# lyndonchan/wsss-analysis

Measured on AMD Instinct MI355X. Metric: images/sec CAM+CRF pseudo-labels, VOC2012 321x321, higher is better.
Workload: dtype f16x3; 1 GPU; resnet50 CAM + dense-CRF (M=21, 10 mean-field iters), 321x321, batch 32 images (=64 samples) per GPU, image-sharded; batch_images=32, num_classes=20, parallelism=image-sharded x1, no collective, steps_per_rank=245

## Files before the change

include/wsscam.h:

```cpp
#ifndef WSSCAM_H
#define WSSCAM_H

#include <stddef.h>
#include <stdint.h>

#ifdef __cplusplus
extern "C" {
#endif

#define WSC_VERSION 100

typedef enum wsc_status {
    WSC_OK = 0,
    WSC_ERR_INVALID = -1,
    WSC_ERR_NO_DEVICE = -2,
    WSC_ERR_HIP = -3,
    WSC_ERR_MISSING_KEY = -4,
    WSC_ERR_SHAPE = -5,
    WSC_ERR_NOMEM = -6,
    WSC_ERR_KEY_RANGE = -7,
    WSC_ERR_CAPACITY = -8,
    WSC_ERR_RANGE = -9
} wsc_status;

typedef enum wsc_arch {
    WSC_ARCH_RESNET50_CAM = 0,
    WSC_ARCH_VGG16_CAM = 1,
    WSC_ARCH_M7_CAM = 2,
    WSC_ARCH_RESNET50_IRN = 3,
    WSC_ARCH_VGG16_IRN = 4,
    WSC_ARCH_M7_IRN = 5
} wsc_arch;

typedef enum wsc_precision {
    WSC_PREC_BF16 = 0,
    WSC_PREC_BF16X3 = 1,
    WSC_PREC_F16 = 2,
    WSC_PREC_F16X3 = 3
} wsc_precision;

typedef struct wsc_ctx wsc_ctx;
typedef struct wsc_net wsc_net;
typedef enum {
    WSC_OPT_CRF_GAUSS_ON_CHIP = 0,
    WSC_OPT_CRF_FUSED_BLUR = 1,
    WSC_OPT_CRF_BLUR_ON_CHIP = 2,
    WSC_OPT_CRF_RANK_BALLOT = 3,
    WSC_OPT_CRF_EMBED_FULL = 4,
    WSC_OPT_RW_TILED = 5,
    WSC_OPT_STEM_POOL_FUSED = 6,
    WSC_OPT_CONV_WINDOW = 7,
    WSC_OPT_CAM_HEAD_STREAM = 8,
    WSC_OPT_CRF_MSG_IN_UPDATE = 9,
    WSC_OPT_COUNT = 10
} wsc_option;

typedef struct wsc_crf wsc_crf;
typedef struct wsc_crf_v wsc_crf_v;

typedef struct wsc_tensor_desc {
    const char *name;
    const float *data;
    int32_t ndim;
    int64_t shape[4];
} wsc_tensor_desc;


int wsc_version(void);
const char *wsc_last_error(void);

int wsc_ctx_create(int device, void *stream, wsc_ctx **out);
void wsc_ctx_destroy(wsc_ctx *ctx);
int wsc_ctx_set_option(wsc_ctx *ctx, int option, int value);
int wsc_sync(wsc_ctx *ctx);
int wsc_ctx_range_status(wsc_ctx *ctx, int *flag_out, int clear);
int wsc_ctx_wait(wsc_ctx *ctx, wsc_ctx *other);
int wsc_ctx_mark(wsc_ctx *ctx, int slot);
int wsc_ctx_wait_mark(wsc_ctx *ctx, int slot);
int wsc_ctx_wait_for_mark(wsc_ctx *ctx, wsc_ctx *other, int slot);
int wsc_device_info(wsc_ctx *ctx, char *arch_name, size_t arch_name_len, int *num_cus);

int wsc_malloc(wsc_ctx *ctx, size_t bytes, void **dptr_out);
int wsc_free(wsc_ctx *ctx, void *dptr);
int wsc_memcpy_h2d(wsc_ctx *ctx, void *dst_dev, const void *src_host, size_t bytes);
int wsc_memcpy_d2h(wsc_ctx *ctx, void *dst_host, const void *src_dev, size_t bytes);
int wsc_memset(wsc_ctx *ctx, void *dst_dev, int value, size_t bytes);
int wsc_host_alloc(wsc_ctx *ctx, size_t bytes, void **host_out);
int wsc_host_free(wsc_ctx *ctx, void *host);
int wsc_host_write_segments(const char *path, int n, const void *const *ptrs, const size_t *sizes);
int wsc_memcpy_h2d_async(wsc_ctx *ctx, void *dst_dev, const void *src_pinned_host, size_t bytes);
int wsc_memcpy_d2h_async(wsc_ctx *ctx, void *dst_pinned_host, const void *src_dev, size_t bytes);

int wsc_timer_begin(wsc_ctx *ctx);
int wsc_timer_end(wsc_ctx *ctx, float *ms_out);

int wsc_profile_begin(wsc_ctx *ctx);
int wsc_profile_end(wsc_ctx *ctx, int max_classes, int32_t *calls_out, float *total_ms_out, double *work_out,
                    int *n_classes_out);
const char *wsc_profile_class_name(int cls);


int wsc_net_create(wsc_ctx *ctx, int arch, const wsc_tensor_desc *weights, int n_weights,
                   int num_classes, int precision, wsc_net **out);
void wsc_net_destroy(wsc_net *net);
int wsc_net_cam_size(const wsc_net *net, int S, int *h_out);
int wsc_net_feat_channels(const wsc_net *net, int *f_out);

int wsc_net_forward_cam(wsc_ctx *ctx, const wsc_net *net, const float *x_dev, int B, int S,
                        float *cam_dev, float *score_dev);
int wsc_net_cam_size_hw(const wsc_net *net, int H, int W, int *h_out, int *w_out);
int wsc_net_forward_cam_hw(wsc_ctx *ctx, const wsc_net *net, const float *x_dev, int B, int H, int W, float *cam_dev,
                           float *score_dev);

int wsc_net_forward_features(wsc_ctx *ctx, const wsc_net *net, const float *x_dev ,
                             int N, int S, float *feat_dev);

int wsc_net_forward_edge(wsc_ctx *ctx, const wsc_net *net, const float *x_dev, int B, int S, int feat_h, int feat_w,
                         float *edge_dev, float *dp_dev);

int wsc_rw_propagate(wsc_ctx *ctx, const float *x_dev, const float *edge_dev, int K, int h, int w,
                     const int32_t *dirs_host, const int32_t *path_start_host, const int32_t *path_yx_host, int D,
                     float beta, int n_steps, float *rw_dev);
int wsc_rw_propagate_batch(wsc_ctx *ctx, int n_img, const int32_t *K_host, const int32_t *h_host,
                           const int32_t *w_host, const float *x_dev, const float *edge_dev,
                           const int32_t *dirs_host, const int32_t *path_start_host, const int32_t *path_yx_host,
                           int D, float beta, int n_steps, float *rw_dev);

int wsc_net_forward_gradcam(wsc_ctx *ctx, const wsc_net *net, const float *x_dev, int N, int S, int relu,
                            float *cams_dev, float *score_dev);

#define WSC_CONV_GENERIC 0x100
int wsc_conv2d_nchw(wsc_ctx *ctx, const float *x_dev, int N, int Cin, int H, int W, const float *w_host,
                    int Cout, int kh, int kw, int stride, int pad, const float *scale_host,
                    const float *shift_host, const float *residual_dev, int relu, int precision,
                    float *y_dev);


// ... 90 lines not shown
```

wsss-analysis_amd/csrc/common.h:

```cpp
#pragma once
#include <hip/hip_runtime.h>
#include <stdint.h>
#include <map>
#include <string>
#include <unordered_map>
#include <vector>

#include "../../include/wsscam.h"

typedef uint16_t bf16_t;

typedef __bf16 bf16x8_t __attribute__((ext_vector_type(8)));
typedef _Float16 f16x8_t __attribute__((ext_vector_type(8)));
typedef float f32x16_t __attribute__((ext_vector_type(16)));
typedef float f32x4_t __attribute__((ext_vector_type(4)));

__host__ __device__ inline bf16_t f32_to_bf16(float f) {
    union { float f; uint32_t u; } v;
    v.f = f;
    uint32_t u = v.u;
    if ((u & 0x7fffffffu) > 0x7f800000u) return (bf16_t)((u >> 16) | 0x40);
    u += 0x7fffu + ((u >> 16) & 1u);
    return (bf16_t)(u >> 16);
}
// ... 28 lines not shown
    }
    return (uint16_t)(o | (sign >> 16));
#endif
}
__host__ __device__ inline float f16_to_f32(uint16_t h) {
#if defined(__HIP_DEVICE_COMPILE__)
    return (float)__builtin_bit_cast(_Float16, h);
#else
    union { float f; uint32_t u; } o, magic;
    magic.u = 113u << 23;
    const uint32_t shifted_exp = 0x7c00u << 13;
    o.u = ((uint32_t)h & 0x7fffu) << 13;
    const uint32_t exp = shifted_exp & o.u;
    o.u += (127u - 15u) << 23;
    if (exp == shifted_exp) o.u += (128u - 16u) << 23;
    else if (exp == 0) { o.u += 1u << 23; o.f -= magic.f; }
    o.u |= ((uint32_t)h & 0x8000u) << 16;
    return o.f;
#endif
}
__host__ __device__ inline uint16_t f32_to_h16(float f, int fmt) { return fmt ? f32_to_f16(f) : f32_to_bf16(f); }
__host__ __device__ inline float h16_to_f32(uint16_t h, int fmt) { return fmt ? f16_to_f32(h) : bf16_to_f32(h); }

void wsc_set_error(const char *fmt, ...);
#define WSC_HIP(expr)                                                                          \
    do {                                                                                       \
        hipError_t _e = (expr);                                                                \
        if (_e != hipSuccess) {                                                                \
            wsc_set_error("%s:%d: %s failed: %s", __FILE__, __LINE__, #expr,                   \
                          hipGetErrorString(_e));                                              \
            return WSC_ERR_HIP;                                                                \
        }                                                                                      \
    } while (0)
#define WSC_CHECK(cond, code, ...)                                                             \
    do {                                                                                       \
        if (!(cond)) {                                                                         \
            wsc_set_error(__VA_ARGS__);                                                        \
            return (code);                                                                     \
        }                                                                                      \
    } while (0)
#define WSC_TRY(expr)                                                                          \
    do {                                                                                       \
        int _s = (expr);                                                                       \
        if (_s != WSC_OK) return _s;                                                           \
    } while (0)

enum WscKernelClass {
    WSC_K_CONV256 = 0,
    WSC_K_CONV128,
    WSC_K_CONV64,
    WSC_K_CONV_SMALLCIN,
    WSC_K_POOL_MISC,
    WSC_K_CAM_TAIL,
    WSC_K_CRF_BUILD,
    WSC_K_GAUSS_MSG,
    WSC_K_BLUR,
    WSC_K_SLICE_UPDATE,
    WSC_K_CRF_MISC,
    WSC_K_COUNT
};
struct WscProfRecord {
    int cls;
    double work;
    hipEvent_t e0, e1;
};

struct wsc_ctx {
    int device = 0;
    hipStream_t stream = nullptr;
    bool own_stream = false;
    int num_cus = 0;
    std::string arch;
    void *ws = nullptr;
    size_t ws_bytes = 0;
    static constexpr int PIN_SLOTS = 8;
    struct PinSlot {
        void *p = nullptr;
        size_t bytes = 0;
        hipEvent_t ev = nullptr;
        bool busy = false;
    };
    PinSlot pin_ring[PIN_SLOTS];
    int pin_next = 0;
    int opt[WSC_OPT_COUNT] = {1, 1, 1, 0, 0, -1, 1, 1, 1, 1};
    void *pinned = nullptr;
    size_t pinned_bytes = 0;
    void *zero_page = nullptr;
    unsigned *range_host = nullptr, *range_dev = nullptr;
    hipEvent_t pinned_ev = nullptr;
    bool pinned_busy = false;
    hipEvent_t ev0 = nullptr, ev1 = nullptr;
    hipEvent_t join_ev = nullptr;
    hipEvent_t marks[8] = {};
    bool mark_set[8] = {};
    hipStream_t aux_stream = nullptr;
    hipEvent_t fork_ev = nullptr, aux_done_ev = nullptr;
    bool profiling = false;
    std::vector<WscProfRecord> prof;
    std::vector<hipEvent_t> prof_pool;
    std::multimap<size_t, void *> free_blocks;
    std::unordered_map<void *, size_t> live_blocks;
    std::vector<std::pair<void *, void (*)(void *)>> attachments;
};
int wsc_ctx_workspace(wsc_ctx *ctx, size_t bytes, void **out);
int wsc_ctx_range_check(wsc_ctx *ctx);
__device__ __forceinline__ unsigned half2_at_ceiling(unsigned hw) { return (hw & 0x7fff7fffu) + 0x04010401u; }
struct WscKernelTimer {
    wsc_ctx *ctx;
    int idx = -1;
    WscKernelTimer(wsc_ctx *c, int cls, double work);
    ~WscKernelTimer();
};
int wsc_ctx_cached_alloc(wsc_ctx *ctx, size_t bytes, void **out);
void wsc_ctx_cached_free(wsc_ctx *ctx, void *p);
struct WscCachedGuard {
    wsc_ctx *ctx;
    void *p;
    WscCachedGuard(wsc_ctx *c, void *q) : ctx(c), p(q) {}
    WscCachedGuard(const WscCachedGuard &) = delete;
    WscCachedGuard &operator=(const WscCachedGuard &) = delete;
    void free_now() {
        if (p) wsc_ctx_cached_free(ctx, p);
        p = nullptr;
    }
    ~WscCachedGuard() { free_now(); }
};
int wsc_ctx_upload_small(wsc_ctx *ctx, void *dst_dev, const void *src_host, size_t bytes);

struct ConvLaunch {
    const bf16_t *x, *x_lo;
    const bf16_t *w;
    const float *s1, *b1;
    const float *s2, *b2;
    const bf16_t *res, *res_lo;
    bf16_t *y, *y_lo;
    float *y_f32;
    int N, H, W, Cin, Ho, Wo, Cout, CoutPad;
    int kh, kw, stride, pad;
    int relu;
    int small_cin;
    int split;
    int fmt;
    int generic;
    int ldy;
    const bf16_t *x2, *x2_lo;
    int H2, W2, C2, stride2;
};
int conv_igemm_launch(wsc_ctx *ctx, const ConvLaunch &p);
int launch_cam_head(wsc_ctx *ctx, const bf16_t *x, const bf16_t *x_lo, int M, int K, const bf16_t *w, int Kw, int CoutPad,
                    const float *s1, const float *b1, int C, int relu, float *y);

int launch_nchw_to_nhwc4(wsc_ctx *ctx, const float *x, int N, int H, int W, bf16_t *y, bf16_t *y_lo, int fmt);
void stem_pool_input_dims(int H, int W, int *Hp, int *Wp);
int launch_stem_pool(wsc_ctx *ctx, const bf16_t *x, const bf16_t *x_lo, int N, int H, int W, const bf16_t *w, int Kw, const float *s1,
                     const float *b1, int relu, bf16_t *y, bf16_t *y_lo);
int launch_gather_strided(wsc_ctx *ctx, const bf16_t *x, const bf16_t *x_lo, int N, int H, int W, int C, int stride, int Ho, int Wo,
                          bf16_t *y, bf16_t *y_lo, int ldy);
int launch_nchw_to_nhwc4_pad(wsc_ctx *ctx, const float *x, int N, int H, int W, int Hp, int Wp, int pad, bf16_t *y, bf16_t *y_lo,
                             int fmt);
int launch_maxpool(wsc_ctx *ctx, const bf16_t *x, const bf16_t *x_lo, int N, int H, int W, int C, int k,
                   int stride, int pad, int Ho, int Wo, bf16_t *y, bf16_t *y_lo, int fmt);
int launch_flip_add(wsc_ctx *ctx, const float *head, int B, int h, int w, int C, int Cs, float *cam);
int launch_gap_linear_sigmoid(wsc_ctx *ctx, const bf16_t *feat, const bf16_t *feat_lo, int B, int hw, int F,
                              const float *Wc, const float *bias, int C, float *score, int fmt,
                              int sample_stride);
int launch_bf16_to_f32(wsc_ctx *ctx, const bf16_t *x, const bf16_t *x_lo, size_t n, float *y, int fmt);
int launch_nchw_to_nhwc(wsc_ctx *ctx, const float *x, int N, int C, int HW, bf16_t *y, bf16_t *y_lo, int fmt);
// ... 12 lines not shown
```

wsss-analysis_amd/csrc/crf.hip:

```cpp
#include "common.h"

#include <atomic>
#include <cmath>
#include <cstring>

namespace {

constexpr unsigned long long EMPTY_KEY = 0xFFFFFFFFFFFFFFFFull;
typedef float f32x2_t __attribute__((ext_vector_type(2)));

struct LatticeDev {
    int d = 0;
    int rep = 1;
    int rows = 0;
    int32_t *offset = nullptr;
    float *bary = nullptr;
    float *norm = nullptr;
    int2 *nbr = nullptr;
    int32_t *tslot_start = nullptr;
    int2 *slot_desc = nullptr;
    float *tent_w = nullptr;
    uint8_t *tent_p = nullptr;
    int32_t *row_slot_start = nullptr;
    int n_tiles = 0, n_slots = 0;
// ... 1646 lines not shown
    const float *sw = T.tent_w + ebase_pix * T.dp1;
    const uint8_t *sp = T.tent_p + ebase_pix * T.dp1;
#pragma unroll
    for (int i = 0; i < EN; ++i) {
        const int e = (int)threadIdx.x + i * (int)blockDim.x;
        r.w[i] = 0.f;
        r.px[i] = 0u;
        if (e < ne) {
            r.w[i] = sw[e];
            r.px[i] = sp[e];
        }
    }
    r.desc = make_int2(0, 0);
    if ((int)threadIdx.x < r.s_end - r.s_beg && threadIdx.x < GATHER_SB) r.desc = T.slot_desc[r.s_beg + threadIdx.x];
}
template <int EN>
__device__ __forceinline__ void splat_commit(const SplatTab &T, int np, const SplatRegs<EN> &r, uint2 *lent, int2 *ldesc, int LP) {
    const int ne = (WSC_SPLAT_ABL & 4) ? 0 : np * T.dp1;
#pragma unroll
    for (int i = 0; i < EN; ++i) {
        const int e = (int)threadIdx.x + i * (int)blockDim.x;
        if (e < ne) lent[e] = make_uint2(r.px[i] * (unsigned)LP, __float_as_uint(r.w[i]));
    }
    if (threadIdx.x < GATHER_SB) ldesc[threadIdx.x] = r.desc;
}
__device__ __forceinline__ void tile_gather(const SplatTab &T, int s_beg, int s_end, int rep_k,
                                            const f32x4_t *stage, uint2 *lent, int2 *ldesc, int LP, int l, int g, int gpw,
                                            bool act) {
    f32x4_t *part = reinterpret_cast<f32x4_t *>(T.part) + (T.shared ? (size_t)rep_k * T.n_slots * LP : (size_t)0);
    const int nw = (int)(blockDim.x >> 6), wv = (int)(threadIdx.x >> 6);
    for (int sb0 = s_beg; sb0 < s_end; sb0 += GATHER_SB) {
        const int nsb = min(GATHER_SB, s_end - sb0);
        if (sb0 > s_beg) {
            if ((int)threadIdx.x < nsb) ldesc[threadIdx.x] = T.slot_desc[sb0 + threadIdx.x];
            __syncthreads();
        }
        for (int s0 = wv * gpw; s0 < nsb; s0 += nw * gpw) {
            const int s = s0 + g;
            const bool ok = act && s < nsb;
            const int2 d = ok ? ldesc[s] : make_int2(0, 0);
            const int i0 = d.x & 0xffff, n = (WSC_SPLAT_ABL & 2) ? 0 : d.x >> 16;
            f32x2_t a01 = {0.f, 0.f}, a23 = {0.f, 0.f};
            const uint2 *le = lent + i0;
            int i = 0;
            for (; i + 4 <= n; i += 4) {
                uint2 en[4];
                f32x4_t in[4];
#pragma unroll
                for (int jj = 0; jj < 4; ++jj) en[jj] = le[i + jj];
#pragma unroll
                for (int jj = 0; jj < 4; ++jj) in[jj] = stage[en[jj].x + l];
#pragma unroll
                for (int jj = 0; jj < 4; ++jj) {
                    const float w = __uint_as_float(en[jj].y);
                    const f32x2_t w2 = {w, w}, lo = {in[jj][0], in[jj][1]}, hi = {in[jj][2], in[jj][3]};
                    a01 = __builtin_elementwise_fma(w2, lo, a01);
                    a23 = __builtin_elementwise_fma(w2, hi, a23);
                }
            }
            if (i < n) {
                uint2 en[3];
                f32x4_t in[3];
#pragma unroll
                for (int jj = 0; jj < 3; ++jj) en[jj] = le[min(i + jj, n - 1)];
#pragma unroll
                for (int jj = 0; jj < 3; ++jj) in[jj] = stage[en[jj].x + l];
#pragma unroll
                for (int jj = 0; jj < 3; ++jj) {
                    const float w = i + jj < n ? __uint_as_float(en[jj].y) : 0.f;
                    const f32x2_t w2 = {w, w}, lo = {in[jj][0], in[jj][1]}, hi = {in[jj][2], in[jj][3]};
                    a01 = __builtin_elementwise_fma(w2, lo, a01);
                    a23 = __builtin_elementwise_fma(w2, hi, a23);
                }
            }
            const f32x4_t acc = {a01[0], a01[1], a23[0], a23[1]};
            if (ok && !(WSC_SPLAT_ABL & 1)) part[(unsigned)d.y * (unsigned)LP + l] = acc;
        }
        __syncthreads();
    }
}

constexpr int REC_LDS_BYTES = 56;
static_assert(TILE_PIX * REC_LDS_BYTES <= (int)(sizeof(uint2) * GATHER_ENT + sizeof(int2) * GATHER_SB), "record stage");
template <bool SLICE, bool SPLAT, bool GF = false, bool DMA = false, int FG = 0>
__global__ __launch_bounds__(512) __attribute__((amdgpu_waves_per_eu(4))) void update_splat_kernel(UpdateArgs a) {
    static_assert(!DMA || (SLICE && GF) || (!SLICE && SPLAT), "the LDS-DMA staging belongs to the GF updates and the first update");
    static_assert(FG == 0 || (SLICE && GF && DMA), "the in-kernel Gaussian message belongs to the DMA-staged GF updates");
    extern __shared__ f32x4_t stage[];
    const int LP = a.LP;
    const int gpw = 64 / LP;
    const int lane = threadIdx.x & 63;
    const int g = lane / LP;
    const int l = lane - g * LP;
    const bool act = g < gpw;
    const int seg0 = g * LP;
    const int nb = gridDim.x, bid = blockIdx.x;
    const int xcd = bid & 7, qq = nb >> 3, rr = nb & 7;
    const int lb = (xcd < rr ? xcd * (qq + 1) : rr * (qq + 1) + (xcd - rr) * qq) + (bid >> 3);
    const int k = lb / a.tg.tpi, j = lb - k * a.tg.tpi;
    const TileBox tb = tile_box(a.tg, j);
    const int np = tb.cw * tb.ch;
    const int N = a.tg.H * a.tg.W;
    const int ppt = (int)(blockDim.x >> 6) * gpw;
    const unsigned cw_magic = tile_div_magic(tb.cw);
    const size_t pix0 = (size_t)k * (size_t)N + (size_t)tb.y0 * (size_t)a.tg.W + (size_t)tb.x0;
    const unsigned LP16 = (unsigned)LP * 16u, l16 = (unsigned)l * 16u;
    constexpr unsigned REC_BYTES = GF ? 52u : 80u;
    constexpr int REC_ID = GF ? 0 : 3, REC_BARY = GF ? 6 : 12, REC_NORM = GF ? 12 : 19;
    const char *rec_b = (GF ? reinterpret_cast<const char *>(a.pix_rec_b) : reinterpret_cast<const char *>(a.pix_rec)) + pix0 * REC_BYTES;
    const char *u_b = reinterpret_cast<const char *>(a.u) + pix0 * LP16;
    char *q_b = reinterpret_cast<char *>(a.q) + pix0 * LP16;
    const char *vg_b = reinterpret_cast<const char *>(a.val_g) + (a.g_rows ? (size_t)k * a.g_rows * LP16 : (size_t)0);
    const char *vb_b = reinterpret_cast<const char *>(a.val_b);
    auto pixel_of = [&](int t0) -> unsigned {
        const int t = t0 + g;
        const unsigned tc = (act && t < np) ? (unsigned)t : 0u;
        const unsigned ty = (tc * cw_magic) >> 16, tx = tc - __umul24(ty, (unsigned)tb.cw);
        return __umul24(ty, (unsigned)a.tg.W) + tx;
    };
    uint4 rq[5];
    f32x4_t unn;
    f32x2_t e01, e23;
    const float cag = a.compat_g * a.alpha_g, cab = a.compat_b * a.alpha_b;
    const char *lrec = reinterpret_cast<const char *>(stage + TILE_PIX * LP);
    auto tile_idx = [&](int t0) -> unsigned {
        const int t = t0 + g;
        return (act && t < np) ? (unsigned)t : 0u;
    };
    auto load_u = [&](int t0) -> f32x4_t {
        if (DMA) return stage[tile_idx(t0) * (unsigned)LP + (unsigned)l];
        return ld_off<f32x4_t>(u_b, __umul24(pixel_of(t0), LP16) + l16);
    };
    auto load_rec = [&](int t0, uint4(&r)[5]) {
        if (DMA) {
            const char *q = lrec + tile_idx(t0) * (unsigned)REC_LDS_BYTES;
            uint2 w[6];
#pragma unroll
            for (int i = 0; i < 6; ++i) w[i] = *reinterpret_cast<const uint2 *>(q + 8 * i);
            r[0] = make_uint4(w[0].x, w[0].y, w[1].x, w[1].y);
            r[1] = make_uint4(w[2].x, w[2].y, w[3].x, w[3].y);
            r[2] = make_uint4(w[4].x, w[4].y, w[5].x, w[5].y);
            r[3] = make_uint4(*reinterpret_cast<const uint32_t *>(q + 48), 0u, 0u, 0u);
            r[4] = make_uint4(0u, 0u, 0u, 0u);
            return;
        }
        const unsigned p = pixel_of(t0);
        if (GF) {
#pragma unroll
            for (int i = 0; i < 3; ++i) r[i] = ld_off<uint4>(rec_b, __umul24(p, REC_BYTES) + 16u * i);
            r[3] = make_uint4(ld_off<uint32_t>(rec_b, __umul24(p, REC_BYTES) + 48u), 0u, 0u, 0u);
            r[4] = make_uint4(0u, 0u, 0u, 0u);
        } else {
#pragma unroll
            for (int i = 0; i < 5; ++i) r[i] = ld_off<uint4>(rec_b, __umul24(p, REC_BYTES) + 16u * i);
        }
    };
    auto issue_rows = [&](const uint4(&r)[5], f32x4_t(&g3)[3], f32x4_t(&b6)[6], float(&w9)[9]) {
        uint32_t rc[20];
#pragma unroll
        for (int i = 0; i < 5; ++i) {
            rc[4 * i] = r[i].x; rc[4 * i + 1] = r[i].y; rc[4 * i + 2] = r[i].z; rc[4 * i + 3] = r[i].w;
        }
        if (!GF) {
#pragma unroll
            for (int i = 0; i < 3; ++i) g3[i] = ld_off<f32x4_t>(vg_b, __umul24(rc[i], LP16) + l16);
        }
#pragma unroll
        for (int i = 0; i < 6; ++i) b6[i] = ld_off<f32x4_t>(vb_b, __umul24(rc[REC_ID + i], LP16) + l16);
        const float wb = cab * __uint_as_float(rc[REC_NORM]);
        if (!GF) {
// ... 180 lines not shown
            for (int it = 0; it < NIT; ++it) {
                const int i = tid + it * GM_THREADS;
                if (i < nitems) gl[i] = o[it];
            }
            __syncthreads();
        }
#pragma unroll
        for (int it = 0; it < NPI; ++it) {
            const int i = tid + it * GM_THREADS;
            if (i < np * LP) {
                const unsigned t = ((unsigned)i * lp_magic) >> 16, ll = (unsigned)i - t * (unsigned)LP;
                const uint4 gp = gpx[it];
                const f32x4_t uu = stage[i];
                f32x2_t o01 = {-uu[0], -uu[1]}, o23 = {-uu[2], -uu[3]};
                const float wr[3] = {__uint_as_float(gp.y) * cag, __uint_as_float(gp.z) * cag, __uint_as_float(gp.w) * cag};
#pragma unroll
                for (int r = 0; r < 3; ++r) {
                    const f32x4_t row = gl[((gp.x >> (10 * r)) & 1023u) * (unsigned)LP + ll];
                    const f32x2_t w2 = {wr[r], wr[r]}, lo = {row[0], row[1]}, hi = {row[2], row[3]};
                    o01 = __builtin_elementwise_fma(w2, lo, o01);
                    o23 = __builtin_elementwise_fma(w2, hi, o23);
                }
                stage[i] = f32x4_t{o01[0], o01[1], o23[0], o23[1]};
            }
        }
        if (SPLAT) splat_fetch<EN_G>(a.sg, a.sg.shared ? j : lb, (a.sg.shared ? 0ll : (long long)k * N) + tb.ebase, np, rg);
        __syncthreads();
    }
    WSC_TL(a, 4);
    auto emit = [&](int t0) {
        const int t = t0 + g;
        const bool ok = act && t < np;
        const unsigned p = pixel_of(t0);
        float e[4] = {e01[0], e01[1], e23[0], e23[1]};
        float mx = -3.0e38f;
#pragma unroll
        for (int kk = 0; kk < 4; ++kk) {
            e[kk] = (ok && 4 * l + kk < a.M) ? e[kk] : -3.0e38f;
            mx = fmaxf(mx, e[kk]);
        }
        for (int o = 4; o > 0; o >>= 1) {
            const float other = __shfl_down(mx, o, 64);
            if (l + o < LP) mx = fmaxf(mx, other);
        }
        mx = __shfl(mx, seg0, 64);
        float ex[4], sum = 0.f;
        const float mxl = mx * 1.44269504088896341f;
#pragma unroll
        for (int kk = 0; kk < 4; ++kk) {
            ex[kk] = __builtin_amdgcn_exp2f(__builtin_fmaf(e[kk], 1.44269504088896341f, -mxl));
            sum += ex[kk];
        }
        for (int o = 4; o > 0; o >>= 1) {
            const float other = __shfl_down(sum, o, 64);
            if (l + o < LP) sum += other;
        }
        sum = __shfl(sum, seg0, 64);
        const float rs = __builtin_amdgcn_rcpf(sum);
        const f32x4_t o4 = {ex[0] * rs, ex[1] * rs, ex[2] * rs, ex[3] * rs};
        if (ok) {
            if (SPLAT) stage[t * LP + l] = o4;
            if (a.q) *reinterpret_cast<f32x4_t *>(q_b + (__umul24(p, LP16) + l16)) = o4;
        }
        if (!SPLAT && a.argmax != nullptr) {
            float bv = o4[0];
            int bi = 4 * l;
#pragma unroll
            for (int kk = 1; kk < 4; ++kk)
                if (4 * l + kk < a.M && o4[kk] > bv) {
                    bv = o4[kk];
                    bi = 4 * l + kk;
                }
            for (int o = 4; o > 0; o >>= 1) {
                const float ov = __shfl_down(bv, o, 64);
                const int oi = __shfl_down(bi, o, 64);
                if (l + o < LP && ov > bv) {
                    bv = ov;
                    bi = oi;
                }
            }
            if (ok && l == 0) a.argmax[pix0 + p] = bi;
        }
    };
    {
        {
            const f32x4_t u0 = load_u(t_first);
            f32x4_t g3[3], b6[6];
            float w9[9];
            if (SLICE) {
                load_rec(t_first, rq);
                issue_rows(rq, g3, b6, w9);
            }
            unn = u0;
            if (t_first + ppt < np) {
                if (SLICE) load_rec(t_first + ppt, rq);
                unn = load_u(t_first + ppt);
            }
            fold(u0, g3, b6, w9, e01, e23);
        }
        for (int t0 = t_first; t0 < np; t0 += ppt) {
            const bool has_next = t0 + ppt < np;
            f32x4_t vgn[3], vbn[6];
            float wrn[9];
            const f32x4_t un1 = unn;
            if (SLICE && has_next) issue_rows(rq, vgn, vbn, wrn);
            if (t0 + 2 * ppt < np) {
                if (SLICE) load_rec(t0 + 2 * ppt, rq);
                unn = load_u(t0 + 2 * ppt);
            }
            emit(t0);
            if (has_next) fold(un1, vgn, vbn, wrn, e01, e23);
        }
    }
    WSC_TL(a, 5);
    if (SPLAT) {
        uint2 *lent = reinterpret_cast<uint2 *>(stage + TILE_PIX * LP);
        int2 *ldesc = reinterpret_cast<int2 *>(lent + GATHER_ENT);
        if (DMA) __syncthreads();
        splat_commit<EN_G>(a.sg, np, rg, lent, ldesc, LP);
        SplatRegs<EN_B> rb;
        splat_fetch<EN_B>(a.sb, a.sb.shared ? j : lb, (a.sb.shared ? 0ll : (long long)k * N) + tb.ebase, np, rb);
        __syncthreads();
        tile_gather(a.sg, rg.s_beg, rg.s_end, k, stage, lent, ldesc, LP, l, g, gpw, act);
        WSC_TL(a, 6);
        splat_commit<EN_B>(a.sb, np, rb, lent, ldesc, LP);
        __syncthreads();
        tile_gather(a.sb, rb.s_beg, rb.s_end, k, stage, lent, ldesc, LP, l, g, gpw, act);
    }
    WSC_TL(a, 7);
}

#ifndef WSC_GF_ABL
#define WSC_GF_ABL 0
#endif
struct GaussMsgArgs {
    const int4 *gt_cnt;
    const int2 *gt_rows;
    const uint4 *gt_nbr;
    const uint4 *gt_pix;
    const float *part;
    const float *u;
    float *e;
    int gt_stride, n_slots, shared, LP, B;
    float cag;
    TileGeom tg;
};
template <int NIT, int NPI>
__global__ __launch_bounds__(GM_THREADS) __attribute__((amdgpu_waves_per_eu(4))) void gauss_msg_kernel(GaussMsgArgs a) {
    extern __shared__ f32x4_t gl[];
    const int LP = a.LP, stride = a.gt_stride, tid = (int)threadIdx.x;
    const f32x4_t zero = {0.f, 0.f, 0.f, 0.f};
    const int nb = gridDim.x, bid = blockIdx.x;
    const int xcd = bid & 7, qq = nb >> 3, rr = nb & 7;
    const int lb = (xcd < rr ? xcd * (qq + 1) : rr * (qq + 1) + (xcd - rr) * qq) + (bid >> 3);
    const int k = lb / a.tg.tpi, j = lb - k * a.tg.tpi;
    const TileBox tb = tile_box(a.tg, j);
    const int np = tb.cw * tb.ch;
    const int N = a.tg.H * a.tg.W;
    unsigned *lnb = reinterpret_cast<unsigned *>(gl + (size_t)stride * (size_t)LP);
    const f32x4_t *partg = reinterpret_cast<const f32x4_t *>(a.part) + (a.shared ? (size_t)k * a.n_slots * LP : (size_t)0);
    const int nitems = stride * LP;
    const unsigned lp_magic = (65536u + (unsigned)LP - 1u) / (unsigned)LP;
    const unsigned cw_magic = tile_div_magic(tb.cw);
    const int2 *trow = a.gt_rows + (size_t)j * stride;
    const uint4 *tn = a.gt_nbr + (size_t)j * stride;
    const unsigned gpix0 = (unsigned)tb.y0 * (unsigned)a.tg.W + (unsigned)tb.x0;
    const size_t pix0 = (size_t)k * (size_t)N + gpix0;
// ... 671 lines not shown
                WSC_HIP(hipStreamSynchronize(ctx->stream));
                WSC_TRY(crf_alloc(crf, sizeof(int2) * nt * GBI * GBJ, (void **)&L.tile_pstart));
                hipLaunchKernelGGL(gauss_tile_pstart_kernel, dim3(grid1d(nt * GBI * GBJ)), dim3(256), 0, ctx->stream,
                                   L.tile_rows, L.row_slot_start, nt * GBI * GBJ, L.tile_pstart);
            }
        }
    }
    float *va, *vb, *vp;
    WSC_TRY(tmp.alloc(sizeof(float) * L.rows, (void **)&va));
    WSC_TRY(tmp.alloc(sizeof(float) * L.rows, (void **)&vb));
    WSC_TRY(tmp.alloc(sizeof(float) * (size_t)(L.n_slots + 1), (void **)&vp));
    splat_ones(ctx, L, make_geom(crf->H, crf->W), va, vp);
    float *res = blur_all1(ctx, L, va, vb);
    uint32_t *rec_b = nullptr;
    if (D == 5 && !shared && crf->lat[0].gt_rows && !crf->pix_rec_b) {
        WSC_TRY(crf_alloc(crf, sizeof(uint32_t) * 13 * (size_t)npix, (void **)&crf->pix_rec_b));
        rec_b = crf->pix_rec_b;
    }
    if (!shared && D == 5) {
        hipLaunchKernelGGL(slice_norm_tile_kernel, dim3((unsigned)L.n_tiles), dim3(256), 0, ctx->stream, L.offset, L.bary, dp1,
                           L.alpha, res, make_geom(crf->H, crf->W), L.norm, rec_b, L.tent_w, L.tent_p);
    } else {
        hipLaunchKernelGGL(slice_norm_kernel, dim3(grid1d(npix)), dim3(256), 0, ctx->stream, L.offset, L.bary, dp1,
                           L.alpha, res, npix, L.norm, rec_b);
        hipLaunchKernelGGL(tile_scale_entries_kernel, dim3((unsigned)L.n_tiles), dim3(256), 0, ctx->stream, L.norm, dp1,
                           make_geom(crf->H, crf->W), L.tent_w, L.tent_p);
    }
    WSC_HIP(hipGetLastError());
    return WSC_OK;
}

struct GaussCache {
    int H, W;
    float sxy;
    LatticeDev L;
    std::vector<void *> blocks;
    int users = 0;
    unsigned long long last_use = 0;
    bool fuse_pending = true;
};
constexpr int GAUSS_CACHE_MAX = 64;
std::atomic<unsigned long long> g_gauss_use_clock{0};
void gauss_cache_delete(void *p) { delete static_cast<GaussCache *>(p); }

int update_threads() {
#ifdef WSC_AB_KNOBS
    const char *te = getenv("WSC_CRF_UPD_THREADS");
    const int nthr = te ? atoi(te) : 256;
    return nthr == 512 ? 512 : 256;
#else
    return 256;
#endif
}
size_t update_splat_lds(int LP) { return sizeof(f32x4_t) * TILE_PIX * LP + sizeof(uint2) * GATHER_ENT + sizeof(int2) * GATHER_SB; }
size_t gauss_msg_lds(int LP, int gt_stride) { return ((size_t)LP * sizeof(f32x4_t) + sizeof(uint4)) * (size_t)gt_stride; }
bool update_gf_ok(const wsc_ctx *ctx, const LatticeDev &G, int LP) {
    if (!ctx->opt[WSC_OPT_CRF_GAUSS_ON_CHIP]) return false;
    if (!G.gt_rows || G.rep < 1 || G.gt_stride <= 0) return false;
    if ((long long)G.gt_stride * LP > 6ll * GM_THREADS || (long long)G.gt_stride * LP >= 8192) return false;
    return gauss_msg_lds(LP, G.gt_stride) <= 64 * 1024;
}

int launch_gauss_msg(wsc_ctx *ctx, hipStream_t st, const GaussMsgArgs &g, double bytes) {
    WscKernelTimer timer(ctx, WSC_K_GAUSS_MSG, bytes);
    const dim3 grid((unsigned)(g.B * g.tg.tpi)), block(GM_THREADS);
    size_t lds = gauss_msg_lds(g.LP, g.gt_stride);
#ifdef WSC_AB_KNOBS
    const char *le = getenv("WSC_CRF_GM_LDS");
    if (le && (size_t)atoi(le) > lds && atoi(le) <= 64 * 1024) lds = (size_t)atoi(le);
#endif
    if ((long long)g.gt_stride * g.LP <= 4ll * GM_THREADS && g.LP <= 6)
        hipLaunchKernelGGL((gauss_msg_kernel<4, 3>), grid, block, lds, st, g);
    else
        hipLaunchKernelGGL((gauss_msg_kernel<6, 4>), grid, block, lds, st, g);
    WSC_HIP(hipGetLastError());
    return WSC_OK;
}

size_t update_fg_lds(int LP, int gt_stride) { return update_splat_lds(LP) + gauss_msg_lds(LP, gt_stride); }
bool update_fg_ok(const wsc_ctx *ctx, const LatticeDev &G, int LP) {
    if (!ctx->opt[WSC_OPT_CRF_MSG_IN_UPDATE] || !update_gf_ok(ctx, G, LP)) return false;
    return update_fg_lds(LP, G.gt_stride) <= 80 * 1024;
}
int launch_update(wsc_ctx *ctx, const UpdateArgs &a, bool slice, bool splat, bool gf, bool fg = false, double fg_bytes = 0.0) {
    const double npix = (double)a.B * a.tg.H * a.tg.W;
    const double by = npix * (2.0 * a.M * 4 + (slice ? (gf ? 6 * 8 + 1.0 * a.M * 4 : 9 * 8 + 2.0 * a.M * 4) : 0.0) +
                              (splat ? 9 * 8 + 2.0 * a.M * 4 : 0.0));
    WscKernelTimer timer(ctx, WSC_K_SLICE_UPDATE, by + (fg ? fg_bytes : 0.0));
    const dim3 grid((unsigned)(a.B * a.tg.tpi)), block(update_threads());
    size_t lds = splat ? update_splat_lds(a.LP) : 0;
    if (fg) {
        const size_t l = update_fg_lds(a.LP, a.gt_stride);
        const bool small = (long long)a.gt_stride * a.LP <= 4ll * GM_THREADS && a.LP <= 6;
        auto set_lds = [&](const void *fn) {
            static bool done[64][4] = {};
            const int dev = ctx->device >= 0 && ctx->device < 64 ? ctx->device : 0, vi = (small ? 0 : 2) + (splat ? 0 : 1);
            if (!done[dev][vi] && l > 48 * 1024) {
                (void)hipFuncSetAttribute(fn, hipFuncAttributeMaxDynamicSharedMemorySize, 96 * 1024);
                done[dev][vi] = true;
            }
        };
        if (small) {
            if (splat) {
                set_lds(reinterpret_cast<const void *>(update_splat_kernel<true, true, true, true, 4>));
                hipLaunchKernelGGL((update_splat_kernel<true, true, true, true, 4>), grid, dim3(GM_THREADS), l, ctx->stream, a);
            } else {
                set_lds(reinterpret_cast<const void *>(update_splat_kernel<true, false, true, true, 4>));
                hipLaunchKernelGGL((update_splat_kernel<true, false, true, true, 4>), grid, dim3(GM_THREADS), l, ctx->stream, a);
            }
        } else {
            if (splat) {
                set_lds(reinterpret_cast<const void *>(update_splat_kernel<true, true, true, true, 6>));
                hipLaunchKernelGGL((update_splat_kernel<true, true, true, true, 6>), grid, dim3(GM_THREADS), l, ctx->stream, a);
            } else {
                set_lds(reinterpret_cast<const void *>(update_splat_kernel<true, false, true, true, 6>));
                hipLaunchKernelGGL((update_splat_kernel<true, false, true, true, 6>), grid, dim3(GM_THREADS), l, ctx->stream, a);
            }
        }
        WSC_HIP(hipGetLastError());
        return WSC_OK;
    }
#ifdef WSC_AB_KNOBS
    const char *de = getenv("WSC_CRF_UPD_DMA");
#else
    const char *de = nullptr;
#endif
    const bool dma = slice && gf && !(de && atoi(de) == 0);
    if (dma) lds = update_splat_lds(a.LP);
    if (dma) {
        if (splat) hipLaunchKernelGGL((update_splat_kernel<true, true, true, true>), grid, block, lds, ctx->stream, a);
        else hipLaunchKernelGGL((update_splat_kernel<true, false, true, true>), grid, block, lds, ctx->stream, a);
    } else if (slice && gf) {
        if (splat) hipLaunchKernelGGL((update_splat_kernel<true, true, true>), grid, block, lds, ctx->stream, a);
        else hipLaunchKernelGGL((update_splat_kernel<true, false, true>), grid, block, lds, ctx->stream, a);
    } else if (slice && splat) hipLaunchKernelGGL((update_splat_kernel<true, true>), grid, block, lds, ctx->stream, a);
    else if (slice) hipLaunchKernelGGL((update_splat_kernel<true, false>), grid, block, lds, ctx->stream, a);
    else if (splat && !(de && atoi(de) == 0))
        hipLaunchKernelGGL((update_splat_kernel<false, true, false, true>), grid, block, lds, ctx->stream, a);
    else if (splat) hipLaunchKernelGGL((update_splat_kernel<false, true>), grid, block, lds, ctx->stream, a);
    else hipLaunchKernelGGL((update_splat_kernel<false, false>), grid, block, lds, ctx->stream, a);
    WSC_HIP(hipGetLastError());
    return WSC_OK;
}

int crf_full_records(wsc_crf *crf, hipStream_t st) {
    if (crf->pix_rec) return WSC_OK;
    wsc_ctx *bctx = crf->ctx;
    WSC_TRY(crf_alloc(crf, sizeof(uint4) * 5 * (size_t)crf->B * crf->N, (void **)&crf->pix_rec));
    if (st != bctx->stream) {
        WSC_HIP(hipEventRecord(bctx->join_ev, bctx->stream));
        WSC_HIP(hipStreamWaitEvent(st, bctx->join_ev, 0));
    }
    hipLaunchKernelGGL(pack_pixels_kernel, dim3((unsigned)grid1d((long long)crf->N * 5, 256, 2048), (unsigned)crf->B), dim3(256), 0, st,
                       crf->lat[0].offset, crf->lat[0].bary, crf->lat[0].norm, crf->lat[1].offset, crf->lat[1].bary,
                       crf->lat[1].norm, crf->N, crf->lat[0].rep > 1 ? 1 : 0, crf->pix_rec);
    WSC_HIP(hipGetLastError());
    return WSC_OK;
}

int crf_bilateral_records(wsc_crf *crf, hipStream_t st) {
    if (crf->pix_rec_b) return WSC_OK;
    wsc_ctx *bctx = crf->ctx;
    WSC_TRY(crf_alloc(crf, sizeof(uint32_t) * 13 * (size_t)crf->B * crf->N, (void **)&crf->pix_rec_b));
    if (st != bctx->stream) {
        WSC_HIP(hipEventRecord(bctx->join_ev, bctx->stream));
        WSC_HIP(hipStreamWaitEvent(st, bctx->join_ev, 0));
    }
    hipLaunchKernelGGL(pack_pixels_b_kernel, dim3((unsigned)grid1d((long long)crf->B * crf->N * 13, 256, 8192)), dim3(256), 0, st,
                       crf->lat[1].offset, crf->lat[1].bary, crf->lat[1].norm, (long long)crf->B * crf->N, crf->pix_rec_b);
    WSC_HIP(hipGetLastError());
    return WSC_OK;
}

}

extern "C" {

int wsc_crf_create(wsc_ctx *ctx, const uint8_t *rgb_dev, int B, int H, int W, float g_sxy, float bi_sxy,
                   float bi_srgb, wsc_crf **out) {
    WSC_CHECK(ctx && rgb_dev && out, WSC_ERR_INVALID, "wsc_crf_create: null argument");
    WSC_CHECK(B > 0 && H > 0 && W > 0, WSC_ERR_INVALID, "wsc_crf_create: B=%d H=%d W=%d", B, H, W);
    WSC_CHECK(g_sxy > 0.f && bi_sxy > 0.f && bi_srgb > 0.f, WSC_ERR_INVALID,
              "wsc_crf_create: kernel widths must be positive");
    WSC_HIP(hipSetDevice(ctx->device));
    wsc_crf *crf = new wsc_crf();
    crf->ctx = ctx; crf->B = B; crf->H = H; crf->W = W; crf->N = H * W;
    WscKernelTimer timer(ctx, WSC_K_CRF_BUILD, (double)B * H * W * (3.0 * 16 + 6.0 * 16));
    int st = WSC_OK;
    GaussCache *hit = nullptr, *lru = nullptr;
    int n_cached = 0;
    size_t lru_at = 0;
    for (size_t i = 0; i < ctx->attachments.size(); ++i) {
        auto &a = ctx->attachments[i];
        if (a.second == &gauss_cache_delete) {
            ++n_cached;
            GaussCache *g = static_cast<GaussCache *>(a.first);
            if (g->H == H && g->W == W && g->sxy == g_sxy) hit = g;
            if (g->users == 0 && (!lru || g->last_use < lru->last_use)) {
                lru = g;
                lru_at = i;
// ... 382 lines not shown
```

wsss-analysis_amd/wsscam/_lib.py:

```python
import ctypes
import os
import re
import threading

import numpy as np

_HERE = os.path.dirname(os.path.abspath(__file__))
LIB_PATH = os.path.join(_HERE, "libwsscam.so")
HEADER_PATH = os.path.normpath(os.path.join(_HERE, "..", "..", "include", "wsscam.h"))

WSC_OK = 0
WSC_ERR_INVALID = -1
WSC_ERR_NO_DEVICE = -2
WSC_ERR_HIP = -3
WSC_ERR_MISSING_KEY = -4
WSC_ERR_SHAPE = -5
WSC_ERR_NOMEM = -6
WSC_ERR_KEY_RANGE = -7
WSC_ERR_CAPACITY = -8
WSC_ERR_RANGE = -9

ARCH_RESNET50_CAM = 0
ARCH_VGG16_CAM = 1
ARCH_M7_CAM = 2
ARCH_RESNET50_IRN = 3
ARCH_VGG16_IRN = 4
ARCH_M7_IRN = 5

PREC_BF16 = 0
PREC_BF16X3 = 1
PREC_F16 = 2
PREC_F16X3 = 3
OPT_CRF_GAUSS_ON_CHIP, OPT_CRF_FUSED_BLUR, OPT_CRF_BLUR_ON_CHIP, OPT_CRF_RANK_BALLOT, OPT_CRF_EMBED_FULL, OPT_RW_TILED, \
    OPT_STEM_POOL_FUSED, OPT_CONV_WINDOW, OPT_CAM_HEAD_STREAM, OPT_CRF_MSG_IN_UPDATE = range(10)
OPT_DEFAULTS = {OPT_CRF_GAUSS_ON_CHIP: 1, OPT_CRF_FUSED_BLUR: 1, OPT_CRF_BLUR_ON_CHIP: 1, OPT_CRF_RANK_BALLOT: 0,
                OPT_CRF_EMBED_FULL: 0, OPT_RW_TILED: -1, OPT_STEM_POOL_FUSED: 1, OPT_CONV_WINDOW: 1, OPT_CAM_HEAD_STREAM: 1,
                OPT_CRF_MSG_IN_UPDATE: 1}
CONV_GENERIC = 0x100


class WscError(RuntimeError):
    def __init__(self, status, message):
        super().__init__("libwsscam error %d: %s" % (status, message))
        self.status = status


class TensorDesc(ctypes.Structure):
    _fields_ = [
        ("name", ctypes.c_char_p),
        ("data", ctypes.POINTER(ctypes.c_float)),
        ("ndim", ctypes.c_int32),
        ("shape", ctypes.c_int64 * 4),
    ]


_lib = None

_vp = ctypes.c_void_p
_i = ctypes.c_int
_f = ctypes.c_float
_sz = ctypes.c_size_t

_SIGNATURES = {
    "wsc_version": (_i, []),
    "wsc_last_error": (ctypes.c_char_p, []),
    "wsc_ctx_create": (_i, [_i, _vp, ctypes.POINTER(_vp)]),
    "wsc_ctx_destroy": (None, [_vp]),
    "wsc_sync": (_i, [_vp]),
    "wsc_ctx_range_status": (_i, [_vp, ctypes.POINTER(_i), _i]),
    "wsc_ctx_wait": (_i, [_vp, _vp]),
    "wsc_ctx_mark": (_i, [_vp, _i]),
    "wsc_ctx_wait_mark": (_i, [_vp, _i]),
    "wsc_ctx_wait_for_mark": (_i, [_vp, _vp, _i]),
    "wsc_device_info": (_i, [_vp, ctypes.c_char_p, _sz, ctypes.POINTER(_i)]),
    "wsc_malloc": (_i, [_vp, _sz, ctypes.POINTER(_vp)]),
    "wsc_free": (_i, [_vp, _vp]),
    "wsc_memcpy_h2d": (_i, [_vp, _vp, _vp, _sz]),
    "wsc_memcpy_d2h": (_i, [_vp, _vp, _vp, _sz]),
    "wsc_memset": (_i, [_vp, _vp, _i, _sz]),
    "wsc_ctx_set_option": (_i, [_vp, _i, _i]),
    "wsc_host_alloc": (_i, [_vp, _sz, ctypes.POINTER(_vp)]),
    "wsc_host_free": (_i, [_vp, _vp]),
    "wsc_host_write_segments": (_i, [ctypes.c_char_p, _i, ctypes.POINTER(_vp), ctypes.POINTER(_sz)]),
    "wsc_memcpy_h2d_async": (_i, [_vp, _vp, _vp, _sz]),
    "wsc_memcpy_d2h_async": (_i, [_vp, _vp, _vp, _sz]),
    "wsc_profile_begin": (_i, [_vp]),
    "wsc_profile_end": (_i, [_vp, _i, _vp, _vp, _vp, ctypes.POINTER(_i)]),
    "wsc_profile_class_name": (ctypes.c_char_p, [_i]),
    "wsc_timer_begin": (_i, [_vp]),
    "wsc_timer_end": (_i, [_vp, ctypes.POINTER(_f)]),
    "wsc_net_create": (_i, [_vp, _i, ctypes.POINTER(TensorDesc), _i, _i, _i, ctypes.POINTER(_vp)]),
    "wsc_net_destroy": (None, [_vp]),
    "wsc_net_cam_size": (_i, [_vp, _i, ctypes.POINTER(_i)]),
    "wsc_net_feat_channels": (_i, [_vp, ctypes.POINTER(_i)]),
    "wsc_net_forward_cam": (_i, [_vp, _vp, _vp, _i, _i, _vp, _vp]),
    "wsc_net_forward_gradcam": (_i, [_vp, _vp, _vp, _i, _i, _i, _vp, _vp]),
    "wsc_net_forward_features": (_i, [_vp, _vp, _vp, _i, _i, _vp]),
    "wsc_net_cam_size_hw": (_i, [_vp, _i, _i, ctypes.POINTER(_i), ctypes.POINTER(_i)]),
    "wsc_net_forward_cam_hw": (_i, [_vp, _vp, _vp, _i, _i, _i, _vp, _vp]),
    "wsc_net_forward_edge": (_i, [_vp, _vp, _vp, _i, _i, _i, _i, _vp, _vp]),
    "wsc_rw_propagate": (_i, [_vp, _vp, _vp, _i, _i, _i, _vp, _vp, _vp, _i, _f, _i, _vp]),
    "wsc_rw_propagate_batch": (_i, [_vp, _i, _vp, _vp, _vp, _vp, _vp, _vp, _vp, _vp, _i, _f, _i, _vp]),
    "wsc_conv2d_nchw": (_i, [_vp, _vp, _i, _i, _i, _i, _vp, _i, _i, _i, _i, _i, _vp, _vp, _vp, _i, _i, _vp]),
    "wsc_cam_postprocess": (_i, [_vp, _vp, _i, _i, _i, _i, _vp, _vp, _vp, _vp, _vp, _vp, _vp]),
    "wsc_cam_eval_confusion": (_i, [_vp, _vp, _i, _vp, _vp, _vp, _vp, _f, _vp, _i, _i, _vp, _vp]),
    "wsc_unary_from_maps": (_i, [_vp, _vp, _i, _i, _i, _f, _vp]),
    "wsc_cam_unary": (_i, [_vp, _vp, _i, _i, _i, _i, _i, _i, _f, _vp]),
    "wsc_cam_unary_pm": (_i, [_vp, _vp, _i, _i, _i, _i, _i, _i, _f, _vp]),
    "wsc_cam_sum_scales": (_i, [_vp, _vp, _i, _i, ctypes.c_longlong, _vp]),
    "wsc_cam_eval_confusion_nn": (_i, [_vp, _vp, _i, _vp, _vp, _vp, _vp, _vp, _vp, _i, _i, _vp, _vp]),
    "wsc_label_confusion_nn": (_i, [_vp, _vp, _i, _vp, _vp, _vp, _vp, _i, _i, _vp, _vp]),
    "wsc_sem_seg_finish": (_i, [_vp, _vp, _i, _vp, _vp, _vp, _vp, _vp, _vp, _i, _f, _vp]),
    "wsc_bilinear_resize": (_i, [_vp, _vp, _i, _i, _i, _vp, _i, _i]),
    "wsc_msf_input_u8": (_i, [_vp, _vp, _i, _vp, _vp, _i, _vp, _vp, _i, _i, _vp]),
    "wsc_resize_u8": (_i, [_vp, _vp, _i, _vp, _vp, _i, _i, _vp]),
    "wsc_label_unary_from_cam": (_i, [_vp, _vp, _i, _i, _i, _f, _f, _vp, _vp]),
    "wsc_ir_label_combine": (_i, [_vp, _vp, _vp, _vp, _i, _i, _i, _vp]),
    "wsc_hsn_gradcam_post": (_i, [_vp, _vp, _i, _i, _i, _i, _i, _vp, _vp, _i, _i]),
    "wsc_hsn_voc_background": (_i, [_vp, _vp, _i, _i, _i, _vp, _i]),
    "wsc_hsn_class_mass": (_i, [_vp, _vp, _i, _i, _vp]),
# ... 683 lines not shown
```

Baseline: 2641 images/s.

## Split CRF update per pixel across two lanes in fused-message kernel

Adds a W2 variant of the fused-message CRF update kernel in which each pixel is handled by a lane pair, each lane owning alternating 4-label chunks. Each lane gathers the six lattice rows and does the softmax and argmax for its chunks, combining max, sum and argmax through xor-shuffles. The aim is to raise per-pixel parallelism and shorten the serial per-thread chain when LP<=6, so one pass covers the whole tile. In exchange it adds shuffle traffic, more per-thread registers for the unrolled row loads, and one more template instantiation. The variant is on by default behind a new option.

```diff
diff --git a/include/wsscam.h b/include/wsscam.h
--- a/include/wsscam.h
+++ b/include/wsscam.h
@@ -52,7 +52,8 @@
     WSC_OPT_CONV_WINDOW = 7,
     WSC_OPT_CAM_HEAD_STREAM = 8,
     WSC_OPT_CRF_MSG_IN_UPDATE = 9,
-    WSC_OPT_COUNT = 10
+    WSC_OPT_CRF_UPDATE_TWO_LANES = 10,
+    WSC_OPT_COUNT = 11
 } wsc_option;
 
 typedef struct wsc_crf wsc_crf;
diff --git a/wsss-analysis_amd/csrc/common.h b/wsss-analysis_amd/csrc/common.h
--- a/wsss-analysis_amd/csrc/common.h
+++ b/wsss-analysis_amd/csrc/common.h
@@ -134,7 +134,7 @@
     };
     PinSlot pin_ring[PIN_SLOTS];
     int pin_next = 0;
-    int opt[WSC_OPT_COUNT] = {1, 1, 1, 0, 0, -1, 1, 1, 1, 1};
+    int opt[WSC_OPT_COUNT] = {1, 1, 1, 0, 0, -1, 1, 1, 1, 1, 1};
     void *pinned = nullptr;
     size_t pinned_bytes = 0;
     void *zero_page = nullptr;
diff --git a/wsss-analysis_amd/csrc/crf.hip b/wsss-analysis_amd/csrc/crf.hip
--- a/wsss-analysis_amd/csrc/crf.hip
+++ b/wsss-analysis_amd/csrc/crf.hip
@@ -1752,10 +1752,12 @@
 
 constexpr int REC_LDS_BYTES = 56;
 static_assert(TILE_PIX * REC_LDS_BYTES <= (int)(sizeof(uint2) * GATHER_ENT + sizeof(int2) * GATHER_SB), "record stage");
-template <bool SLICE, bool SPLAT, bool GF = false, bool DMA = false, int FG = 0>
+static_assert(2 * TILE_PIX <= GM_THREADS, "W2: one trip covers the tile");
+template <bool SLICE, bool SPLAT, bool GF = false, bool DMA = false, int FG = 0, bool W2 = false>
 __global__ __launch_bounds__(512) __attribute__((amdgpu_waves_per_eu(4))) void update_splat_kernel(UpdateArgs a) {
     static_assert(!DMA || (SLICE && GF) || (!SLICE && SPLAT), "the LDS-DMA staging belongs to the GF updates and the first update");
     static_assert(FG == 0 || (SLICE && GF && DMA), "the in-kernel Gaussian message belongs to the DMA-staged GF updates");
+    static_assert(!W2 || FG > 0, "the two-lane trips belong to the FG variants (GM_THREADS threads, E and records in LDS)");
     extern __shared__ f32x4_t stage[];
     const int LP = a.LP;
     const int gpw = 64 / LP;
@@ -2102,7 +2104,118 @@
             if (ok && l == 0) a.argmax[pix0 + p] = bi;
         }
     };
-    {
+    if constexpr (W2) {
+        const unsigned h = threadIdx.x & 1u;
+        const int t = (int)(threadIdx.x >> 1);
+        const bool ok = t < np;
+        const unsigned tc = ok ? (unsigned)t : 0u;
+        const int nu = (LP - (int)h + 1) >> 1;
+        const unsigned ty = __umul24(tc, cw_magic) >> 16, tx = tc - __umul24(ty, (unsigned)tb.cw);
+        const unsigned p = __umul24(ty, (unsigned)a.tg.W) + tx;
+        const unsigned s0 = __umul24(tc, (unsigned)LP) + h;
+        const char *rp = lrec + __umul24(tc, (unsigned)REC_LDS_BYTES);
+        uint2 rw[6];
+#pragma unroll
+        for (int i = 0; i < 6; ++i) rw[i] = *reinterpret_cast<const uint2 *>(rp + 8 * i);
+        const float wb = cab * __uint_as_float(*reinterpret_cast<const uint32_t *>(rp + 48));
+        const uint32_t id[6] = {rw[0].x, rw[0].y, rw[1].x, rw[1].y, rw[2].x, rw[2].y};
+        const uint32_t by[6] = {rw[3].x, rw[3].y, rw[4].x, rw[4].y, rw[5].x, rw[5].y};
+        unsigned ro[6];
+        float wr[6];
+#pragma unroll
+        for (int r = 0; r < 6; ++r) {
+            ro[r] = __umul24(id[r], LP16) + h * 16u;
+            wr[r] = __uint_as_float(by[r]) * wb;
+        }
+        f32x4_t rows[3][6];
+#pragma unroll
+        for (int i = 0; i < 3; ++i)
+            if (i < nu) {
+#pragma unroll
+                for (int r = 0; r < 6; ++r) rows[i][r] = ld_off<f32x4_t>(vb_b + 32 * i, ro[r]);
+            }
+        float e[3][4];
+#pragma unroll
+        for (int i = 0; i < 3; ++i) {
+#pragma unroll
+            for (int kk = 0; kk < 4; ++kk) e[i][kk] = -3.0e38f;
+            if (i < nu) {
+                const f32x4_t u = stage[s0 + 2u * i];
+                f32x2_t o01 = {u[0], u[1]}, o23 = {u[2], u[3]};
+#pragma unroll
+                for (int r = 0; r < 6; ++r) {
+                    const f32x2_t w2 = {wr[r], wr[r]}, lo = {rows[i][r][0], rows[i][r][1]}, hi = {rows[i][r][2], rows[i][r][3]};
+                    o01 = __builtin_elementwise_fma(w2, lo, o01);
+                    o23 = __builtin_elementwise_fma(w2, hi, o23);
+                }
+                const float ev[4] = {o01[0], o01[1], o23[0], o23[1]};
+                const int c0 = 4 * ((int)h + 2 * i);
+#pragma unroll
+                for (int kk = 0; kk < 4; ++kk) e[i][kk] = (ok && c0 + kk < a.M) ? ev[kk] : -3.0e38f;
+            }
+        }
+        float mx = -3.0e38f;
+#pragma unroll
+        for (int i = 0; i < 3; ++i)
+#pragma unroll
+            for (int kk = 0; kk < 4; ++kk) mx = fmaxf(mx, e[i][kk]);
+        mx = fmaxf(mx, __shfl_xor(mx, 1, 64));
+        const float mxl = mx * 1.44269504088896341f;
+        float ex[3][4], s[3];
+#pragma unroll
+        for (int i = 0; i < 3; ++i) {
+            s[i] = 0.f;
+#pragma unroll
+            for (int kk = 0; kk < 4; ++kk) {
+                ex[i][kk] = __builtin_amdgcn_exp2f(__builtin_fmaf(e[i][kk], 1.44269504088896341f, -mxl));
+                s[i] += ex[i][kk];
+            }
+        }
+        float sum = s[0];
+        if (nu > 2) sum += s[2];
+        if (nu > 1) sum += s[1];
+        if (LP > 1) sum += __shfl_xor(sum, 1, 64);
+        const float rs = __builtin_amdgcn_rcpf(sum);
+        f32x4_t o4[3];
+#pragma unroll
+        for (int i = 0; i < 3; ++i) {
+            o4[i] = f32x4_t{ex[i][0] * rs, ex[i][1] * rs, ex[i][2] * rs, ex[i][3] * rs};
+            if (ok && i < nu) {
+                if (SPLAT) stage[s0 + 2u * i] = o4[i];
+                if (a.q) *reinterpret_cast<f32x4_t *>(q_b + (__umul24(p, LP16) + h * 16u + 32u * i)) = o4[i];
+            }
+        }
+        if (!SPLAT && a.argmax != nullptr) {
+            float bv[3];
+            int bi[3];
+#pragma unroll
+            for (int i = 0; i < 3; ++i) {
+                const int c0 = 4 * ((int)h + 2 * i);
+                bv[i] = o4[i][0];
+                bi[i] = c0;
+#pragma unroll
+                for (int kk = 1; kk < 4; ++kk)
+                    if (c0 + kk < a.M && o4[i][kk] > bv[i]) {
+                        bv[i] = o4[i][kk];
+                        bi[i] = c0 + kk;
+                    }
+            }
+            float v = bv[0];
+            int ci = bi[0];
+            if (nu > 2 && bv[2] > v) {
+                v = bv[2];
+                ci = bi[2];
+            }
+            if (nu > 1 && bv[1] > v) {
+                v = bv[1];
+                ci = bi[1];
+            }
+            const float ov = __shfl_xor(v, 1, 64);
+            const int oi = __shfl_xor(ci, 1, 64);
+            if (LP > 1 && ov > v) ci = oi;
+            if (ok && h == 0) a.argmax[pix0 + p] = ci;
+        }
+    } else {
         {
             const f32x4_t u0 = load_u(t_first);
             f32x4_t g3[3], b6[6];
@@ -2940,6 +3053,17 @@
     if (!ctx->opt[WSC_OPT_CRF_MSG_IN_UPDATE] || !update_gf_ok(ctx, G, LP)) return false;
     return update_fg_lds(LP, G.gt_stride) <= 80 * 1024;
 }
+template <bool SPLAT, int FG, bool W2>
+void launch_update_fg(wsc_ctx *ctx, const UpdateArgs &a, dim3 grid, size_t lds) {
+    static bool done[64] = {};
+    const int dev = ctx->device >= 0 && ctx->device < 64 ? ctx->device : 0;
+    if (!done[dev] && lds > 48 * 1024) {
+        (void)hipFuncSetAttribute(reinterpret_cast<const void *>(update_splat_kernel<true, SPLAT, true, true, FG, W2>),
+                                  hipFuncAttributeMaxDynamicSharedMemorySize, 96 * 1024);
+        done[dev] = true;
+    }
+    hipLaunchKernelGGL((update_splat_kernel<true, SPLAT, true, true, FG, W2>), grid, dim3(GM_THREADS), lds, ctx->stream, a);
+}
 int launch_update(wsc_ctx *ctx, const UpdateArgs &a, bool slice, bool splat, bool gf, bool fg = false, double fg_bytes = 0.0) {
     const double npix = (double)a.B * a.tg.H * a.tg.W;
     const double by = npix * (2.0 * a.M * 4 + (slice ? (gf ? 6 * 8 + 1.0 * a.M * 4 : 9 * 8 + 2.0 * a.M * 4) : 0.0) +
@@ -2950,30 +3074,13 @@
     if (fg) {
         const size_t l = update_fg_lds(a.LP, a.gt_stride);
         const bool small = (long long)a.gt_stride * a.LP <= 4ll * GM_THREADS && a.LP <= 6;
-        auto set_lds = [&](const void *fn) {
-            static bool done[64][4] = {};
-            const int dev = ctx->device >= 0 && ctx->device < 64 ? ctx->device : 0, vi = (small ? 0 : 2) + (splat ? 0 : 1);
-            if (!done[dev][vi] && l > 48 * 1024) {
-                (void)hipFuncSetAttribute(fn, hipFuncAttributeMaxDynamicSharedMemorySize, 96 * 1024);
-                done[dev][vi] = true;
-            }
-        };
+        const bool w2 = ctx->opt[WSC_OPT_CRF_UPDATE_TWO_LANES] && a.LP <= 6;
         if (small) {
-            if (splat) {
-                set_lds(reinterpret_cast<const void *>(update_splat_kernel<true, true, true, true, 4>));
-                hipLaunchKernelGGL((update_splat_kernel<true, true, true, true, 4>), grid, dim3(GM_THREADS), l, ctx->stream, a);
-            } else {
-                set_lds(reinterpret_cast<const void *>(update_splat_kernel<true, false, true, true, 4>));
-                hipLaunchKernelGGL((update_splat_kernel<true, false, true, true, 4>), grid, dim3(GM_THREADS), l, ctx->stream, a);
-            }
+            if (w2) splat ? launch_update_fg<true, 4, true>(ctx, a, grid, l) : launch_update_fg<false, 4, true>(ctx, a, grid, l);
+            else splat ? launch_update_fg<true, 4, false>(ctx, a, grid, l) : launch_update_fg<false, 4, false>(ctx, a, grid, l);
         } else {
-            if (splat) {
-                set_lds(reinterpret_cast<const void *>(update_splat_kernel<true, true, true, true, 6>));
-                hipLaunchKernelGGL((update_splat_kernel<true, true, true, true, 6>), grid, dim3(GM_THREADS), l, ctx->stream, a);
-            } else {
-                set_lds(reinterpret_cast<const void *>(update_splat_kernel<true, false, true, true, 6>));
-                hipLaunchKernelGGL((update_splat_kernel<true, false, true, true, 6>), grid, dim3(GM_THREADS), l, ctx->stream, a);
-            }
+            if (w2) splat ? launch_update_fg<true, 6, true>(ctx, a, grid, l) : launch_update_fg<false, 6, true>(ctx, a, grid, l);
+            else splat ? launch_update_fg<true, 6, false>(ctx, a, grid, l) : launch_update_fg<false, 6, false>(ctx, a, grid, l);
         }
         WSC_HIP(hipGetLastError());
         return WSC_OK;
diff --git a/wsss-analysis_amd/wsscam/_lib.py b/wsss-analysis_amd/wsscam/_lib.py
--- a/wsss-analysis_amd/wsscam/_lib.py
+++ b/wsss-analysis_amd/wsscam/_lib.py
@@ -32,10 +32,10 @@
 PREC_F16 = 2
 PREC_F16X3 = 3
 OPT_CRF_GAUSS_ON_CHIP, OPT_CRF_FUSED_BLUR, OPT_CRF_BLUR_ON_CHIP, OPT_CRF_RANK_BALLOT, OPT_CRF_EMBED_FULL, OPT_RW_TILED, \
-    OPT_STEM_POOL_FUSED, OPT_CONV_WINDOW, OPT_CAM_HEAD_STREAM, OPT_CRF_MSG_IN_UPDATE = range(10)
+    OPT_STEM_POOL_FUSED, OPT_CONV_WINDOW, OPT_CAM_HEAD_STREAM, OPT_CRF_MSG_IN_UPDATE, OPT_CRF_UPDATE_TWO_LANES = range(11)
 OPT_DEFAULTS = {OPT_CRF_GAUSS_ON_CHIP: 1, OPT_CRF_FUSED_BLUR: 1, OPT_CRF_BLUR_ON_CHIP: 1, OPT_CRF_RANK_BALLOT: 0,
                 OPT_CRF_EMBED_FULL: 0, OPT_RW_TILED: -1, OPT_STEM_POOL_FUSED: 1, OPT_CONV_WINDOW: 1, OPT_CAM_HEAD_STREAM: 1,
-                OPT_CRF_MSG_IN_UPDATE: 1}
+                OPT_CRF_MSG_IN_UPDATE: 1, OPT_CRF_UPDATE_TWO_LANES: 1}
 CONV_GENERIC = 0x100
 
 
```

Result: faster. 2673 images/s, median of 6 (+1.2%).
